# rohitgandikota/sliders

Hardware: AMD Instinct MI355X
Metric: UNet denoise steps/sec (SDXL rank-4 text slider) (higher is better)
Workload: dtype bf16; 1 GPU; sdxl text slider rank=4 alpha=1 noxattn+c3lier, 1024x1024, batch 1 (CFG pair), DDIM-50 partial denoise k~U{1..49} + 4 predictions + backward + AdamW; bench_step=one training iteration, prompt_pairs=8, parallelism=dp1

## Files before the change

### sliders_amd/csrc/lora.hip

```cpp
#include "common.h"
#include "../../include/sliders_hip.h"

namespace {

struct AddrArgs {
    const __bf16* a0; const __bf16* a1;
    int lda0, lda1, ca0, ca1;
    int mode, hs, ws, src_xform, stride, ho, wo;
};

template <int RMAX, int LPR>
__global__ __launch_bounds__(256) void skinny_kernel(AddrArgs A, const __bf16* __restrict__ w,
                                                     const __bf16* __restrict__ bias, void* out,
                                                     int M, int R, int K, int ldo, int out_kind, int kmajor) {
    const int tid = threadIdx.x;
    const int sub = tid & (LPR - 1);
    const int m = blockIdx.x * (256 / LPR) + tid / LPR;
    const bool active = m < M;
    const int mm = active ? m : M - 1;
    float acc[RMAX];
#pragma unroll
    for (int r = 0; r < RMAX; ++r) acc[r] = 0.f;
    const int cin = A.ca0 + A.ca1;

// ... 7 lines not shown
                for (int h = 0; h < 4; ++h) {
                    const bf16x8 wv = *(const bf16x8*)(w + (long)k * 4 + h * 8);
#pragma unroll
                    for (int r = 0; r < 4; ++r) {
                        acc[r] += xf[2 * h] * (float)wv[r];
                        acc[r] += xf[2 * h + 1] * (float)wv[4 + r];
                    }
                }
            }
            return;
        }
        bf16x8 wv[RMAX];
#pragma unroll
        for (int r = 0; r < RMAX; ++r) wv[r] = *(const bf16x8*)(w + (long)(r < R ? r : 0) * K + k);
#pragma unroll
        for (int r = 0; r < RMAX; ++r) {
            if (r < R) {
#pragma unroll
                for (int e = 0; e < 8; ++e) acc[r] += xf[e] * (float)wv[r][e];
            }
        }
    };

    if (A.mode == 0) {
        auto src_of = [&](int k) {
            const int kc = k < K ? k : 0;
            return kc < A.ca0 ? A.a0 + (long)mm * A.lda0 + kc : A.a1 + (long)mm * A.lda1 + (kc - A.ca0);
        };
        bf16x8 cur = *(const bf16x8*)src_of(sub * 8);
        for (int k = sub * 8; k < K; k += LPR * 8) {
            const bf16x8 nxt = *(const bf16x8*)src_of(k + LPR * 8);
            fma_chunk(cur, k);
            cur = nxt;
        }
    } else {
        const int hw = A.ho * A.wo;
        const int b = mm / hw;
        const int rem = mm - b * hw;
        const int oy = rem / A.wo, ox = rem - oy * A.wo;
        const int sh = A.src_xform ? 1 : 0;
        const int HL = A.hs << sh, WL = A.ws << sh;
        for (int tap = 0; tap < 9; ++tap) {
            const int ky = tap / 3, kx = tap - ky * 3;
            const int iy = oy * A.stride + ky - 1, ix = ox * A.stride + kx - 1;
            bool ok = (iy >= 0) & (iy < HL) & (ix >= 0) & (ix < WL);
            if (A.src_xform == 2) ok = ok & (((iy | ix) & 1) == 0);
            if (!ok) continue;
            const long pix = ((long)b * A.hs + (iy >> sh)) * A.ws + (ix >> sh);
            auto src_of = [&](int c) {
                const int cc = c < cin ? c : 0;
                return cc < A.ca0 ? A.a0 + pix * A.lda0 + cc : A.a1 + pix * A.lda1 + (cc - A.ca0);
            };
            bf16x8 cur = *(const bf16x8*)src_of(sub * 8);
            for (int c = sub * 8; c < cin; c += LPR * 8) {
                const bf16x8 nxt = *(const bf16x8*)src_of(c + LPR * 8);
                fma_chunk(cur, tap * cin + c);
                cur = nxt;
            }
        }
    }
#pragma unroll
    for (int r = 0; r < RMAX; ++r) {
#pragma unroll
        for (int o = LPR / 2; o > 0; o >>= 1) acc[r] += __shfl_xor(acc[r], o, 64);
    }
    if (active && sub == 0) {
        if (out_kind == 0) {
            float* o = (float*)out + (long)m * ldo;
#pragma unroll
            for (int r = 0; r < RMAX; ++r)
                if (r < R) o[r] = acc[r] + (bias ? (float)bias[r] : 0.f);
        } else {
            const int hw = A.ho * A.wo;
            const int b = m / hw;
            const int rem = m - b * hw;
            __bf16* o = (__bf16*)out;
#pragma unroll
            for (int r = 0; r < RMAX; ++r)
                if (r < R) o[((long)b * R + r) * hw + rem] = (__bf16)(acc[r] + (bias ? (float)bias[r] : 0.f));
        }
    }
}

__global__ __launch_bounds__(256) void gemv_kernel(const slh_gemv_desc d) {
    const int lane = threadIdx.x & 63;
    const int n = blockIdx.x * 4 + (threadIdx.x >> 6);
    if (n >= d.N) return;
    const __bf16* x = (const __bf16*)d.x;
    const __bf16* w = (const __bf16*)d.w + (long)n * d.K;
    float acc[8];
#pragma unroll
    for (int b = 0; b < 8; ++b) acc[b] = 0.f;
    for (int k = lane * 8; k < d.K; k += 512) {
        const bf16x8 wv = *(const bf16x8*)(w + k);
        bf16x8 xv[8];
#pragma unroll
        for (int b = 0; b < 8; ++b) xv[b] = *(const bf16x8*)(x + (long)(b < d.nb ? b : d.nb - 1) * d.ldx + k);
        float wf[8];
#pragma unroll
        for (int e = 0; e < 8; ++e) wf[e] = (float)wv[e];
#pragma unroll
        for (int b = 0; b < 8; ++b) {
            if (b < d.nb) {
#pragma unroll
                for (int e = 0; e < 8; ++e) {
                    float xe = (float)xv[b][e];
                    if (d.in_act == 1) xe = round_bf16(silu_f(xe));
                    acc[b] += xe * wf[e];
                }
            }
        }
    }
#pragma unroll
    for (int b = 0; b < 8; ++b) acc[b] = wave_sum(acc[b]);
    if (lane == 0) {
        const float bias = d.bias ? (float)((const __bf16*)d.bias)[n] : 0.f;
        float up[4] = {0.f, 0.f, 0.f, 0.f};
        float ls = 0.f;
        int tcol = 0;
        if (d.lora_t) {
            ls = *d.lora_scale;
            tcol = d.lora_tcol ? d.lora_tcol[n] : 0;
            const bf16x4 u = *(const bf16x4*)((const __bf16*)d.lora_up + (long)n * 4);
#pragma unroll
            for (int r = 0; r < 4; ++r) up[r] = (float)u[r];
        }
        for (int b = 0; b < d.nb; ++b) {
            float v = acc[b] + bias;
            if (d.lora_t) {
                const float* t = d.lora_t + (long)b * d.ld_t + tcol;
                v += ls * (t[0] * up[0] + t[1] * up[1] + t[2] * up[2] + t[3] * up[3]);
            }
            if (d.addend) v = round_bf16(v) + (float)((const __bf16*)d.addend)[(long)b * d.ld_add + n];
            if (d.out_f32) ((float*)d.y)[(long)b * d.ldy + n] = v;
            else ((__bf16*)d.y)[(long)b * d.ldy + n] = (__bf16)v;
        }
    }
}

struct WgradArgs {
    AddrArgs A;
    const float* v; float* out; const float* scale;
    int M, R, ldv, ldo, rows_per_block, rmajor, vgroup_cols;
    float* ws; unsigned* ticket;
};

template <int R>
__device__ __forceinline__ void wgrad_body(const WgradArgs& p, const int bx, const int by, const int bz, const long slab_id = 0,
                                           const int slab_step = 0, const long ticket_id = 0, const int splits = 1) {
    __shared__ float red[4][32][8 * R + 1];
    __shared__ int last_flag;
    const int cx = threadIdx.x & 31, ry = threadIdx.x >> 5;
    const int C = p.A.ca0 + p.A.ca1;
    const int c = (bx * 32 + cx) * 8;
    const bool cvalid = c < C;
    const int tap = bz;
    const int m_begin = by * p.rows_per_block;
    const int m_end = min(p.M, m_begin + p.rows_per_block);
    float acc[8][R];
#pragma unroll
    for (int e = 0; e < 8; ++e)
#pragma unroll
        for (int r = 0; r < R; ++r) acc[e][r] = 0.f;
    const int voff = p.vgroup_cols > 0 ? 4 * (c / p.vgroup_cols) : 0;
    const int sh = p.A.src_xform ? 1 : 0;
    const int HL = p.A.hs << sh, WL = p.A.ws << sh;
    const int ky = tap / 3, kx = tap - ky * 3;
    const int hw = p.A.ho * p.A.wo;
    if (cvalid) {
        for (int m = m_begin + ry; m < m_end; m += 8) {
            const __bf16* src;
            if (p.A.mode == 0) {
                src = c < p.A.ca0 ? p.A.a0 + (long)m * p.A.lda0 + c : p.A.a1 + (long)m * p.A.lda1 + (c - p.A.ca0);
            } else {
                const int b = m / hw;
                const int rem = m - b * hw;
                const int oy = rem / p.A.wo, ox = rem - oy * p.A.wo;
                const int iy = oy * p.A.stride + ky - 1, ix = ox * p.A.stride + kx - 1;
                bool ok = (iy >= 0) & (iy < HL) & (ix >= 0) & (ix < WL);
                if (p.A.src_xform == 2) ok = ok & (((iy | ix) & 1) == 0);
                if (!ok) continue;
                const long pix = ((long)b * p.A.hs + (iy >> sh)) * p.A.ws + (ix >> sh);
                src = c < p.A.ca0 ? p.A.a0 + pix * p.A.lda0 + c : p.A.a1 + pix * p.A.lda1 + (c - p.A.ca0);
            }
            const bf16x8 z = *(const bf16x8*)src;
            float vv[R];
#pragma unroll
            for (int r = 0; r < R; ++r) vv[r] = p.v[(long)m * p.ldv + voff + r];
#pragma unroll
            for (int e = 0; e < 8; ++e) {
                const float ze = (float)z[e];
#pragma unroll
                for (int r = 0; r < R; ++r) acc[e][r] += ze * vv[r];
            }
        }
    }
#pragma unroll
    for (int e = 0; e < 8; ++e)
#pragma unroll
        for (int r = 0; r < R; ++r) {
            acc[e][r] += __shfl_xor(acc[e][r], 32, 64);
            if ((threadIdx.x & 32) == 0) red[threadIdx.x >> 6][cx][e * R + r] = acc[e][r];
        }
    __syncthreads();
    const float s = *p.scale;
    if (p.ws != nullptr) {
        constexpr int PER = 32 * 8 * R;
        const __amdgpu_buffer_rsrc_t slabs = __builtin_amdgcn_make_buffer_rsrc(p.ws + slab_id * PER - (long)by * slab_step * PER, 0,
                                                                              (int)((long)splits * slab_step * PER * 4), 0x00020000);
#pragma unroll
        for (int q = 0; q < PER / 1024; ++q) {
            const int idx = (q * 256 + threadIdx.x) * 4;
            f32x4 t4;
#pragma unroll
            for (int u = 0; u < 4; ++u) {
                const int ccx = (idx + u) / (8 * R), er = (idx + u) - ccx * (8 * R);
                float t = 0.f;
#pragma unroll
// ... 45 lines not shown
    }
}

template <int R>
__global__ __launch_bounds__(256) void wgrad_kernel(const WgradArgs p) {
    wgrad_body<R>(p, blockIdx.x, blockIdx.y, blockIdx.z, ((long)blockIdx.z * gridDim.y + blockIdx.y) * gridDim.x + blockIdx.x,
                  (int)gridDim.x, (long)blockIdx.z * gridDim.x + blockIdx.x, (int)gridDim.y);
}

struct WgradGeom { int gx, splits, taps, rows_per_block; };
__host__ __device__ inline WgradGeom wgrad_geom(int C, int M, int mode, int kind) {
    WgradGeom g;
    g.gx = (C / 8 + 31) / 32;
    g.taps = mode == 1 ? 9 : 1;
    const int blocks_xz = g.gx * g.taps;
    const int target = kind == 0 ? 768 : 256;
    int splits = kind == 2 ? (M + 511) / 512 : (target + blocks_xz - 1) / blocks_xz;
    const int max_splits = (M + 63) / 64, min_splits = kind == 2 ? 1 : (M + 1023) / 1024;
    if (splits > max_splits) splits = max_splits;
    if (splits < min_splits) splits = min_splits;
    if (splits < 1) splits = 1;
    g.splits = splits;
    g.rows_per_block = ((M + splits - 1) / splits + 7) / 8 * 8;
    return g;
}

__host__ __device__ inline void wgrad_args(WgradArgs& p, const slh_wgrad_desc& d) {
    p.A.a0 = (const __bf16*)d.z0; p.A.a1 = (const __bf16*)d.z1;
    p.A.lda0 = d.ldz0; p.A.lda1 = d.ldz1; p.A.ca0 = d.c0; p.A.ca1 = d.c1; p.A.mode = d.mode;
    p.A.hs = d.hs; p.A.ws = d.ws; p.A.src_xform = d.src_xform; p.A.stride = d.stride; p.A.ho = d.ho; p.A.wo = d.wo;
    p.v = d.v; p.out = d.out; p.scale = d.scale;
    p.M = d.M; p.R = d.R; p.ldv = d.ldv; p.ldo = d.ldo;
    p.rmajor = d.out_rmajor;
    p.vgroup_cols = d.vgroup_cols;
    p.ws = d.slabs; p.ticket = (unsigned*)d.tickets;
    p.rows_per_block = wgrad_geom(d.c0 + d.c1, d.M, d.mode, d.slabs ? 1 : 0).rows_per_block;
}

__device__ __forceinline__ int batch_find(const int* prefix, int n, int bid) {
    int lo = 0, hi = n;
    while (hi - lo > 1) {
        const int mid = (lo + hi) >> 1;
        if (prefix[mid] <= bid) lo = mid; else hi = mid;
    }
    return lo;
}

template <int R>
__global__ __launch_bounds__(256) void wgrad_batch_kernel(const slh_wgrad_desc* table, const int* prefix, int n, float* ws, unsigned* ticket) {
    const int bid = blockIdx.x;
    const int pi = __builtin_amdgcn_readfirstlane(batch_find(prefix, n, bid));
    const slh_wgrad_desc d = table[pi];
    WgradArgs p;
    wgrad_args(p, d);
    p.ws = ws; p.ticket = ticket;
    const WgradGeom g = wgrad_geom(d.c0 + d.c1, d.M, d.mode, ws ? 2 : 0);
    p.rows_per_block = g.rows_per_block;
    const int local = bid - prefix[pi];
    const int bx = local % g.gx, rest = local / g.gx;
    const int by = rest % g.splits, bz = rest / g.splits;
    wgrad_body<R>(p, bx, by, bz, bid, g.gx, (long)prefix[pi] + (long)bz * g.splits * g.gx + bx, g.splits);
}

}

static int fill_addr(AddrArgs& A, const void* a0, const void* a1, int lda0, int lda1, int ca0, int ca1, int mode,
                     int hs, int ws, int src_xform, int stride, int ho, int wo) {
    A.a0 = (const __bf16*)a0; A.a1 = (const __bf16*)a1;
    A.lda0 = lda0; A.lda1 = lda1; A.ca0 = ca0; A.ca1 = ca1; A.mode = mode;
    A.hs = hs; A.ws = ws; A.src_xform = src_xform; A.stride = stride; A.ho = ho; A.wo = wo;
    return 0;
}

struct skinny_form { int rmax, lpr, grid; };
static skinny_form skinny_choose(int M, int R) {
    skinny_form f;
    f.rmax = R <= 4 ? 4 : R <= 12 ? 12 : 16;
    f.lpr = M <= 16384 ? 64 : 16;
    const int rows = 256 / f.lpr;
    f.grid = (M + rows - 1) / rows;
    return f;
}

extern "C" int slh_skinny(const slh_skinny_desc* d, slh_stream_t stream) {
    SLH_CHECK(d && d->a0 && d->w && d->out, "slh_skinny: null pointer");
    SLH_CHECK(d->M > 0 && d->R > 0 && d->R <= 16 && d->K > 0, "slh_skinny: bad shape");
    SLH_CHECK(d->ca0 % 8 == 0 && d->ca1 % 8 == 0 && d->lda0 % 8 == 0 && d->lda1 % 8 == 0 && d->K % 8 == 0,
              "slh_skinny: 16-byte alignment");
    SLH_CHECK((d->a1 != nullptr) == (d->ca1 > 0), "slh_skinny: a1/ca1 mismatch");
    const int cin = d->ca0 + d->ca1;
    if (d->mode == 0) SLH_CHECK(cin == d->K, "slh_skinny: dense K mismatch");
    else {
        SLH_CHECK(d->mode == 1 && d->K == 9 * cin, "slh_skinny: conv K mismatch");
        SLH_CHECK(d->M == d->batch * d->ho * d->wo, "slh_skinny: conv M mismatch");
        SLH_CHECK(d->stride == 1 || d->stride == 2, "slh_skinny: stride");
    }
    if (d->out_kind == 1) SLH_CHECK(d->mode == 1, "slh_skinny: NCHW output needs conv geometry");
    if (d->w_kmajor) SLH_CHECK(d->R == 4 && d->mode == 0 && !d->bias, "slh_skinny: w_kmajor needs dense R=4");
    AddrArgs A;
    fill_addr(A, d->a0, d->a1, d->lda0, d->lda1, d->ca0, d->ca1, d->mode, d->hs, d->ws, d->src_xform, d->stride,
              d->ho, d->wo);
    hipStream_t s = (hipStream_t)stream;
    const skinny_form f = skinny_choose(d->M, d->R);
#define SLH_SKINNY_LAUNCH(RM, LPR)                                                                                 \
    do {                                                                                                           \
        if (slh_name_mode()) slh_name_record("skinny<%d,%d>", RM, LPR);                                            \
        else                                                                                                       \
            hipLaunchKernelGGL((skinny_kernel<RM, LPR>), dim3(f.grid), dim3(256), 0, s, A, (const __bf16*)d->w,    \
                               (const __bf16*)d->bias, d->out, d->M, d->R, d->K, d->ldo, d->out_kind, d->w_kmajor); \
    } while (0)
#define SLH_SKINNY_ROWS(RM)                                                                                        \
    do {                                                                                                           \
        if (f.lpr == 64) SLH_SKINNY_LAUNCH(RM, 64);                                                                \
        else SLH_SKINNY_LAUNCH(RM, 16);                                                                            \
    } while (0)
    if (f.rmax == 4) SLH_SKINNY_ROWS(4);
    else if (f.rmax == 12) SLH_SKINNY_ROWS(12);
    else SLH_SKINNY_ROWS(16);
#undef SLH_SKINNY_ROWS
#undef SLH_SKINNY_LAUNCH
    SLH_LAUNCH_CHECK("slh_skinny");
    return 0;
}

extern "C" int slh_skinny_kernel_name(const slh_skinny_desc* d, char* buf, int cap) {
    SLH_CHECK(buf && cap >= 32, "slh_skinny_kernel_name: buffer");
    slh_name_sink_set(buf, cap);
    const int rc = slh_skinny(d, nullptr);
    slh_name_sink_set(nullptr, 0);
    if (rc == 0 && !buf[0]) { slh_set_error("slh_skinny_kernel_name: internal: no launch site recorded a name"); return -3; }
    return rc;
}

extern "C" int slh_gemv(const slh_gemv_desc* d, slh_stream_t stream) {
    SLH_CHECK(d && d->x && d->w && d->y, "slh_gemv: null pointer");
    SLH_CHECK(d->nb >= 1 && d->nb <= 8 && d->N > 0 && d->K > 0 && d->K % 8 == 0 && d->ldx % 8 == 0,
              "slh_gemv: bad shape nb=%d N=%d K=%d", d->nb, d->N, d->K);
    if (d->lora_t) SLH_CHECK(d->lora_up && d->lora_scale, "slh_gemv: lora pointers");
    hipLaunchKernelGGL(gemv_kernel, dim3((d->N + 3) / 4), dim3(256), 0, (hipStream_t)stream, *d);
    SLH_LAUNCH_CHECK("slh_gemv");
    return 0;
}

static int wgrad_check(const slh_wgrad_desc* d, bool ptrs = true) {
    SLH_CHECK(d, "slh_lora_wgrad: null descriptor");
    if (ptrs) SLH_CHECK(d->z0 && d->v && d->out && d->scale, "slh_lora_wgrad: null pointer");
    SLH_CHECK(d->R == 4 || d->R == 12, "slh_lora_wgrad: R must be 4 or 12");
    SLH_CHECK(d->c0 % 8 == 0 && d->c1 % 8 == 0 && d->ldz0 % 8 == 0 && d->ldz1 % 8 == 0, "slh_lora_wgrad: alignment");
    if (ptrs) SLH_CHECK((d->z1 != nullptr) == (d->c1 > 0), "slh_lora_wgrad: z1/c1 mismatch");
    SLH_CHECK(d->M > 0 && d->c0 + d->c1 > 0, "slh_lora_wgrad: empty problem");
    if (d->mode == 1) SLH_CHECK(d->M == d->batch * d->ho * d->wo, "slh_lora_wgrad: conv M mismatch");
    if (d->vgroup_cols > 0)
        SLH_CHECK(d->vgroup_cols % 8 == 0 && (d->c0 + d->c1) % d->vgroup_cols == 0 && d->R == 4,
                  "slh_lora_wgrad: vgroup_cols %d needs a multiple of 8 that divides C = %d, and R = 4 (R = %d)", d->vgroup_cols,
                  d->c0 + d->c1, d->R);
    SLH_CHECK(d->vgroup_cols >= 0, "slh_lora_wgrad: negative vgroup_cols");
    return 0;
}

extern "C" int slh_lora_wgrad(const slh_wgrad_desc* d, slh_stream_t stream) {
    if (wgrad_check(d)) return -1;
    WgradArgs p;
    wgrad_args(p, *d);
    SLH_CHECK((d->slabs != nullptr) == (d->tickets != nullptr), "slh_lora_wgrad: slabs and tickets come together");
    const WgradGeom g = wgrad_geom(d->c0 + d->c1, d->M, d->mode, d->slabs ? 1 : 0);
    dim3 grid(g.gx, g.splits, g.taps);
    hipStream_t s = (hipStream_t)stream;
    if (d->R == 4) hipLaunchKernelGGL(wgrad_kernel<4>, grid, dim3(256), 0, s, p);
    else hipLaunchKernelGGL(wgrad_kernel<12>, grid, dim3(256), 0, s, p);
    SLH_LAUNCH_CHECK("slh_lora_wgrad");
    return 0;
}

extern "C" int slh_lora_wgrad_blocks(const slh_wgrad_desc* d) {
    if (wgrad_check(d, false)) return -1;
    const WgradGeom g = wgrad_geom(d->c0 + d->c1, d->M, d->mode, d->slabs ? 2 : 0);
    return g.gx * g.splits * g.taps;
}

extern "C" int slh_lora_wgrad_single_blocks(const slh_wgrad_desc* d) {
    if (wgrad_check(d, false)) return -1;
    const WgradGeom g = wgrad_geom(d->c0 + d->c1, d->M, d->mode, 1);
    return g.gx * g.splits * g.taps;
}

extern "C" int slh_lora_wgrad_geometry(const slh_wgrad_desc* d, int kind, int32_t* out4) {
    if (wgrad_check(d, false)) return -1;
    SLH_CHECK(kind >= 0 && kind <= 2 && out4, "slh_lora_wgrad_geometry: kind must be 0, 1 or 2");
    const WgradGeom g = wgrad_geom(d->c0 + d->c1, d->M, d->mode, kind);
    out4[0] = g.gx; out4[1] = g.splits; out4[2] = g.taps; out4[3] = g.rows_per_block;
    return 0;
}

extern "C" int slh_lora_wgrad_batch(const slh_batch_desc* d, slh_stream_t stream) {
    SLH_CHECK(d && d->table && d->prefix && d->n > 0 && d->total > 0, "slh_lora_wgrad_batch: empty batch / null pointer");
    SLH_CHECK(d->arg == 4 || d->arg == 12, "slh_lora_wgrad_batch: arg must be the common R (4 or 12)");
    SLH_CHECK((d->slabs != nullptr) == (d->tickets != nullptr), "slh_lora_wgrad_batch: slabs and tickets come together");
    hipStream_t s = (hipStream_t)stream;
    if (d->arg == 4)
        hipLaunchKernelGGL(wgrad_batch_kernel<4>, dim3(d->total), dim3(256), 0, s, (const slh_wgrad_desc*)d->table, d->prefix, d->n,
                           (float*)d->slabs, (unsigned*)d->tickets);
    else
        hipLaunchKernelGGL(wgrad_batch_kernel<12>, dim3(d->total), dim3(256), 0, s, (const slh_wgrad_desc*)d->table, d->prefix, d->n,
                           (float*)d->slabs, (unsigned*)d->tickets);
    SLH_LAUNCH_CHECK("slh_lora_wgrad_batch");
    return 0;
}

namespace {
__global__ __launch_bounds__(256) void lora_conv_dgrad_kernel(const slh_lora_cdgrad_desc d) {
    const int nchunk = d.cin / 8;
    const long gid = (long)blockIdx.x * blockDim.x + threadIdx.x;
    const long total = (long)d.batch * d.hl * d.wl * nchunk;
    if (gid >= total) return;
    const int chunk = (int)(gid % nchunk);
    const long pix = gid / nchunk;
    const int hw = d.hl * d.wl;
    const int b = (int)(pix / hw);
    const int rem = (int)(pix - (long)b * hw);
    const int iy = rem / d.wl, ix = rem - iy * d.wl;
    const int c = chunk * 8;
    const __bf16* A = (const __bf16*)d.a_down;
// ... 117 lines not shown
```

### sliders_amd/csrc/ops.hip

```cpp
#include "common.h"
#include "../../include/sliders_hip.h"

namespace {

__global__ void tembed_kernel(const slh_tembed_desc d) {
    const int idx = blockIdx.x * blockDim.x + threadIdx.x;
    const int per = d.n_vals * d.dim;
    if (idx >= d.nb * per) return;
    const int b = idx / per;
    const int rem = idx - b * per;
    const int j = rem / d.dim;
    const int i = rem - j * d.dim;
    const int half = d.dim / 2;
    const int fi = i < half ? i : i - half;
    const float exponent = (-9.210340371976184f * (float)fi) / (float)half;
    const float arg = d.vals[b * d.n_vals + j] * expf(exponent);
    const float v = i < half ? cosf(arg) : sinf(arg);
    ((__bf16*)d.out)[(long)b * d.ldo + d.col0 + rem] = (__bf16)v;
}

constexpr int CONVIN_ITERS = 8;
__global__ void conv_in_kernel(const slh_convin_desc d, int nchunk, int ppb) {
    extern __shared__ __attribute__((aligned(16))) char cin_smem[];
    __bf16* sw = (__bf16*)cin_smem;
    const int K = 9 * d.cin;
    for (int i = threadIdx.x; i < K * d.cout; i += blockDim.x) {
        const int co = i / K, k = i - co * K;
        sw[k * d.cout + co] = ((const __bf16*)d.w)[i];
    }
    __syncthreads();
    const int chunk = threadIdx.x % nchunk, pl = threadIdx.x / nchunk;
    const int hw = d.h * d.wd;
    const long npix = (long)d.batch * hw;
    float bias[8];
#pragma unroll
    for (int e = 0; e < 8; ++e) bias[e] = d.bias ? (float)((const __bf16*)d.bias)[chunk * 8 + e] : 0.f;
    for (int it = 0; it < CONVIN_ITERS; ++it) {
        const long pix = ((long)blockIdx.x * CONVIN_ITERS + it) * ppb + pl;
        if (pix >= npix) break;
        const int b = (int)(pix / hw);
        const int rem = (int)(pix - (long)b * hw);
        const int oy = rem / d.wd, ox = rem - oy * d.wd;
        const __bf16* x = (const __bf16*)d.x + (long)b * d.cin * hw;
        float acc[8];
#pragma unroll
        for (int e = 0; e < 8; ++e) acc[e] = bias[e];
        if (d.cin <= 4) {
            __bf16 xin[9][4];
            bool tin[9];
#pragma unroll
            for (int tap = 0; tap < 9; ++tap) {
                const int iy = oy + tap / 3 - 1, ix = ox + tap % 3 - 1;
                tin[tap] = iy >= 0 && iy < d.h && ix >= 0 && ix < d.wd;
                const int cy = iy < 0 ? 0 : (iy >= d.h ? d.h - 1 : iy), cx = ix < 0 ? 0 : (ix >= d.wd ? d.wd - 1 : ix);
#pragma unroll
                for (int ci = 0; ci < 4; ++ci) xin[tap][ci] = x[(long)(ci < d.cin ? ci : 0) * hw + cy * d.wd + cx];
            }
#pragma unroll
            for (int tap = 0; tap < 9; ++tap) {
                if (!tin[tap]) continue;
#pragma unroll
                for (int ci = 0; ci < 4; ++ci) {
                    if (ci >= d.cin) break;
                    const float xv = (float)xin[tap][ci];
                    const bf16x8 wv = *(const bf16x8*)(sw + (tap * d.cin + ci) * d.cout + chunk * 8);
#pragma unroll
                    for (int e = 0; e < 8; ++e) acc[e] += xv * (float)wv[e];
                }
            }
        } else {
            for (int tap = 0; tap < 9; ++tap) {
                const int iy = oy + tap / 3 - 1, ix = ox + tap % 3 - 1;
                if (iy < 0 || iy >= d.h || ix < 0 || ix >= d.wd) continue;
                for (int ci = 0; ci < d.cin; ++ci) {
                    const float xv = (float)x[(long)ci * hw + iy * d.wd + ix];
                    const bf16x8 wv = *(const bf16x8*)(sw + (tap * d.cin + ci) * d.cout + chunk * 8);
#pragma unroll
                    for (int e = 0; e < 8; ++e) acc[e] += xv * (float)wv[e];
                }
            }
        }
        bf16x8 o;
#pragma unroll
        for (int e = 0; e < 8; ++e) o[e] = (__bf16)acc[e];
        *(bf16x8*)((__bf16*)d.y + pix * d.ldy + chunk * 8) = o;
    }
}

__global__ __launch_bounds__(256) void ew_kernel(const slh_ew_desc d) {
    const int nchunk = d.C / 8;
    const long gid = (long)blockIdx.x * blockDim.x + threadIdx.x;
    if (gid >= (long)d.M * nchunk) return;
    const int chunk = (int)(gid % nchunk);
    const long m = gid / nchunk;
    const int c = chunk * 8;
    const __bf16* A = (const __bf16*)d.a;
    const __bf16* B = (const __bf16*)d.b;
    __bf16* O = (__bf16*)d.out;
    if (d.op == SLH_EW_COPY) {
        *(bf16x8*)(O + m * d.ldo + c) = *(const bf16x8*)(A + m * d.lda + c);
    } else if (d.op == SLH_EW_ADD) {
        const bf16x8 x = *(const bf16x8*)(A + m * d.lda + c);
        const bf16x8 y = *(const bf16x8*)(B + m * d.ldb + c);
        bf16x8 o;
#pragma unroll
        for (int e = 0; e < 8; ++e) o[e] = (__bf16)((float)x[e] + (float)y[e]);
        *(bf16x8*)(O + m * d.ldo + c) = o;
    } else if (d.op == SLH_EW_GEGLU_FWD || d.op == SLH_EW_GEGLU_BWD) {
        const int jb = c >> 5, j = c & 31;
        const __bf16* pa = A + m * d.lda + jb * 64 + j;
        const bf16x8 hv = *(const bf16x8*)pa;
        const bf16x8 gv = *(const bf16x8*)(pa + 32);
        if (d.op == SLH_EW_GEGLU_FWD) {
            bf16x8 o;
#pragma unroll
            for (int e = 0; e < 8; ++e) o[e] = (__bf16)((float)hv[e] * round_bf16(gelu_erf_fast_f((float)gv[e])));
            *(bf16x8*)(O + m * d.ldo + c) = o;
        } else {
            const bf16x8 dy = *(const bf16x8*)(B + m * d.ldb + c);
            bf16x8 dh, dg;
#pragma unroll
            for (int e = 0; e < 8; ++e) {
                const float g = (float)gv[e], hh = (float)hv[e], dd = (float)dy[e];
                const float cdf = 0.5f * (1.f + erff(g * 0.70710678118654752f));
                const float pdf = 0.3989422804014327f * __expf(-0.5f * g * g);
                dh[e] = (__bf16)(dd * round_bf16(g * cdf));
                dg[e] = (__bf16)(round_bf16(dd * hh) * (cdf + g * pdf));
            }
            __bf16* po = O + m * d.ldo + jb * 64 + j;
            *(bf16x8*)po = dh;
            *(bf16x8*)(po + 32) = dg;
        }
    } else if (d.op == SLH_EW_UPSAMPLE_BWD) {
        const int w = d.iarg, hw = d.iarg2;
        const long b = m / hw;
        const int rem = (int)(m - b * hw);
        const int y = rem / w, x = rem - y * w;
        const long base = (b * 4 * hw + (long)(2 * y) * (2 * w) + 2 * x);
        float acc[8];
#pragma unroll
        for (int e = 0; e < 8; ++e) acc[e] = 0.f;
#pragma unroll
        for (int q = 0; q < 4; ++q) {
            const long row = base + (q >> 1) * (2 * w) + (q & 1);
            const bf16x8 v = *(const bf16x8*)(A + row * d.lda + c);
#pragma unroll
            for (int e = 0; e < 8; ++e) acc[e] += (float)v[e];
        }
        bf16x8 o;
#pragma unroll
        for (int e = 0; e < 8; ++e) o[e] = (__bf16)acc[e];
        *(bf16x8*)(O + m * d.ldo + c) = o;
    }
}

__global__ __launch_bounds__(256) void colsum_kernel(const slh_ew_desc d) {
    __shared__ float red[8][33][8];
    const int cx = threadIdx.x & 31, ry = threadIdx.x >> 5;
    const int c = (blockIdx.x * 32 + cx) * 8;
    const int hw = d.iarg2;
    const int b = blockIdx.z;
    const int r0 = blockIdx.y * 512, r1 = min(hw, r0 + 512);
    float acc[8];
#pragma unroll
    for (int e = 0; e < 8; ++e) acc[e] = 0.f;
    if (c < d.C) {
        for (int r = r0 + ry; r < r1; r += 8) {
            const bf16x8 v = *(const bf16x8*)((const __bf16*)d.a + ((long)b * hw + r) * d.lda + c);
// ... 69 lines not shown
        }
    }
    sq = wave_sum(sq);
    __shared__ float part[16];
    if ((threadIdx.x & 63) == 0) part[threadIdx.x >> 6] = sq;
    __syncthreads();
    if (threadIdx.x == 0) {
        float t = 0.f;
#pragma unroll
        for (int w = 0; w < 16; ++w) t += part[w];
        *d.loss += t / (float)d.n;
    }
}

__global__ __launch_bounds__(256) void adamw_kernel(const slh_adamw_desc d, float decay, float bc2_sqrt,
                                                    float step_size, float w1, float beta2, float w2, float eps) {
    const long i = (long)blockIdx.x * blockDim.x + threadIdx.x;
    if (i >= d.n) return;
    __bf16* P = (__bf16*)d.param; __bf16* M1 = (__bf16*)d.exp_avg; __bf16* M2 = (__bf16*)d.exp_avg_sq;
    const float g = round_bf16(d.grad[i] * d.grad_scale);
    float p = round_bf16((float)P[i] * decay);
    float m = (float)M1[i];
    m = round_bf16(m + w1 * (g - m));
    float v = round_bf16((float)M2[i] * beta2);
    v = round_bf16(v + w2 * (g * g));
    float den = round_bf16(sqrtf(v));
    den = round_bf16(den / bc2_sqrt);
    den = round_bf16(den + eps);
    p = round_bf16(p + (-step_size) * (m / den));
    P[i] = (__bf16)p; M1[i] = (__bf16)m; M2[i] = (__bf16)v;
}

__global__ __launch_bounds__(256) void adamw_f32_kernel(const slh_adamw_desc d, float decay, float bc2_sqrt,
                                                        float neg_step_size, float w1, float beta2, float w2, float eps) {
    const long i = (long)blockIdx.x * blockDim.x + threadIdx.x;
    if (i >= d.n) return;
    float* P = (float*)d.param; float* M1 = (float*)d.exp_avg; float* M2 = (float*)d.exp_avg_sq;
    const float g = d.grad_scale == 1.0f ? d.grad[i] : d.grad[i] * d.grad_scale;
    float p = P[i] * decay;
    float m = M1[i];
    m = __builtin_fmaf(w1, g - m, m);
    float v = M2[i] * beta2;
    v = __builtin_fmaf(w2, g * g, v);
    float den = __builtin_sqrtf(v);
    den = den / bc2_sqrt;
    den = den + eps;
    p = __builtin_fmaf(neg_step_size, m / den, p);
    P[i] = p; M1[i] = m; M2[i] = v;
    ((__bf16*)d.param_lo)[i] = (__bf16)p;
}

__global__ __launch_bounds__(256) void lion_kernel(const slh_lion_desc d, float decay, float b1, float w1, float b2,
                                                   float w2, float neg_lr) {
    const long i = (long)blockIdx.x * blockDim.x + threadIdx.x;
    if (i >= d.n) return;
    __bf16* P = (__bf16*)d.param; __bf16* M = (__bf16*)d.exp_avg;
    const float g = round_bf16(d.grad[i] * d.grad_scale);
    float p = round_bf16((float)P[i] * decay);
    const float m0 = (float)M[i];
    float u = round_bf16(m0 * b1);
    u = round_bf16(u + w1 * g);
    const float sg = u > 0.f ? 1.f : (u < 0.f ? -1.f : 0.f);
    p = round_bf16(p + neg_lr * sg);
    float m = round_bf16(m0 * b2);
    m = round_bf16(m + w2 * g);
    P[i] = (__bf16)p; M[i] = (__bf16)m;
}

}

extern "C" int slh_timestep_embed(const slh_tembed_desc* d, slh_stream_t stream) {
    SLH_CHECK(d && d->vals && d->out && d->dim % 2 == 0 && d->nb > 0 && d->n_vals > 0, "slh_timestep_embed: bad desc");
    const int total = d->nb * d->n_vals * d->dim;
    hipLaunchKernelGGL(tembed_kernel, dim3((total + 255) / 256), dim3(256), 0, (hipStream_t)stream, *d);
    SLH_LAUNCH_CHECK("slh_timestep_embed");
    return 0;
}

extern "C" int slh_conv_in(const slh_convin_desc* d, slh_stream_t stream) {
    SLH_CHECK(d && d->x && d->w && d->y, "slh_conv_in: null pointer");
    SLH_CHECK(d->cout % 8 == 0 && d->ldy % 8 == 0 && d->cin > 0 && d->cin <= 16, "slh_conv_in: bad shape");
    const int nchunk = d->cout / 8;
    SLH_CHECK(nchunk <= 256 && 9 * d->cin * d->cout * 2 <= 64 * 1024, "slh_conv_in: weights must fit 64 KB of LDS");
    const int ppb = 256 / nchunk;
    const long npix = (long)d->batch * d->h * d->wd;
    const long per_block = (long)ppb * CONVIN_ITERS;
    hipLaunchKernelGGL(conv_in_kernel, dim3((unsigned)((npix + per_block - 1) / per_block)), dim3(nchunk * ppb),
                       9 * d->cin * d->cout * 2, (hipStream_t)stream, *d, nchunk, ppb);
    SLH_LAUNCH_CHECK("slh_conv_in");
    return 0;
}

extern "C" int slh_elementwise(const slh_ew_desc* d, slh_stream_t stream) {
    SLH_CHECK(d && d->a && d->out, "slh_elementwise: null pointer");
    SLH_CHECK(d->C % 8 == 0 && d->lda % 8 == 0 && d->ldo % 4 == 0, "slh_elementwise: alignment");
    hipStream_t s = (hipStream_t)stream;
    if (d->op == SLH_EW_COLSUM) {
        SLH_CHECK(d->iarg2 > 0 && d->M % d->iarg2 == 0, "slh_elementwise: colsum rows per sample");
        dim3 grid((d->C / 8 + 31) / 32, (d->iarg2 + 511) / 512, d->M / d->iarg2);
        hipLaunchKernelGGL(colsum_kernel, grid, dim3(256), 0, s, *d);
    } else {
        if (d->op == SLH_EW_ADD || d->op == SLH_EW_GEGLU_BWD) SLH_CHECK(d->b && d->ldb % 8 == 0, "slh_elementwise: operand b");
        if (d->op == SLH_EW_GEGLU_FWD || d->op == SLH_EW_GEGLU_BWD) SLH_CHECK(d->C % 32 == 0, "slh_elementwise: geglu C");
        if (d->op == SLH_EW_UPSAMPLE_BWD) SLH_CHECK(d->iarg > 0 && d->iarg2 > 0, "slh_elementwise: upsample dims");
        const long total = (long)d->M * (d->C / 8);
        hipLaunchKernelGGL(ew_kernel, dim3((unsigned)((total + 255) / 256)), dim3(256), 0, s, *d);
    }
    SLH_LAUNCH_CHECK("slh_elementwise");
    return 0;
}

namespace {
__global__ __launch_bounds__(256) void gather16_kernel(const unsigned short* src, const int* idx, unsigned short* out, long n) {
    const long i = (long)blockIdx.x * blockDim.x + threadIdx.x;
    if (i >= n) return;
    const int j = idx[i];
    out[i] = j < 0 ? (unsigned short)0 : src[j];
}
}

extern "C" int slh_gather16(const slh_gather16_desc* d, slh_stream_t stream) {
    SLH_CHECK(d && d->src && d->idx && d->out && d->n > 0, "slh_gather16: null pointer / empty");
    hipLaunchKernelGGL(gather16_kernel, dim3((unsigned)((d->n + 255) / 256)), dim3(256), 0, (hipStream_t)stream,
                       (const unsigned short*)d->src, d->idx, (unsigned short*)d->out, (long)d->n);
    SLH_LAUNCH_CHECK("slh_gather16");
    return 0;
}

extern "C" int slh_cfg_ddim(const slh_cfg_ddim_desc* d, slh_stream_t stream) {
    SLH_CHECK(d && d->eps && d->out && (d->x || !d->do_step), "slh_cfg_ddim: null pointer");
    const long n = (long)d->nb * d->chw;
    hipLaunchKernelGGL(cfg_ddim_kernel, dim3((unsigned)((n + 255) / 256)), dim3(256), 0, (hipStream_t)stream, *d);
    SLH_LAUNCH_CHECK("slh_cfg_ddim");
    return 0;
}

extern "C" int slh_guidance_loss(const slh_loss_desc* d, slh_stream_t stream) {
    SLH_CHECK(d && d->target && d->positive && d->neutral && d->uncond && d->loss, "slh_guidance_loss: null pointer");
    hipLaunchKernelGGL(loss_kernel, dim3(1), dim3(1024), 0, (hipStream_t)stream, *d);
    SLH_LAUNCH_CHECK("slh_guidance_loss");
    return 0;
}

extern "C" int slh_adamw(const slh_adamw_desc* d, slh_stream_t stream) {
    SLH_CHECK(d && d->param && d->exp_avg && d->exp_avg_sq && d->grad && d->step >= 1, "slh_adamw: bad desc");
    const double bc1 = 1.0 - pow(d->beta1, (double)d->step);
    const double bc2 = 1.0 - pow(d->beta2, (double)d->step);
    const float step_size = (float)(d->lr / bc1);
    const float bc2_sqrt = (float)sqrt(bc2);
    const float decay = (float)(1.0 - d->lr * d->weight_decay);
    if (d->f32_state) {
        SLH_CHECK(d->param_lo && ((uintptr_t)d->param & 3) == 0, "slh_adamw: f32_state needs param_lo (the bf16 copy the kernels read)");
        hipLaunchKernelGGL(adamw_f32_kernel, dim3((unsigned)((d->n + 255) / 256)), dim3(256), 0, (hipStream_t)stream, *d,
                           decay, bc2_sqrt, -step_size, (float)(1.0 - d->beta1), (float)d->beta2, (float)(1.0 - d->beta2), (float)d->eps);
        SLH_LAUNCH_CHECK("slh_adamw (fp32 state)");
        return 0;
    }
    hipLaunchKernelGGL(adamw_kernel, dim3((unsigned)((d->n + 255) / 256)), dim3(256), 0, (hipStream_t)stream, *d,
                       decay, bc2_sqrt, step_size, (float)(1.0 - d->beta1), (float)d->beta2, (float)(1.0 - d->beta2),
                       (float)d->eps);
    SLH_LAUNCH_CHECK("slh_adamw");
    return 0;
}

extern "C" int slh_lion(const slh_lion_desc* d, slh_stream_t stream) {
    SLH_CHECK(d && d->param && d->exp_avg && d->grad && d->n > 0, "slh_lion: bad desc");
// ... 7 lines not shown
```

Baseline: 44.98 steps/s.

## Add MFMA kernels for LoRA skinny conv and conv_in, retune GEMV

Adds an MFMA-based kernel for the rank-4 LoRA down-projection over 3x3 conv inputs. It stages padded weights in LDS and prefetches the next channel chunk into registers. It also adds an MFMA path for the 4-channel conv_in layer, with weights and bias held in registers. The GEMV kernel is templated on batch count and rows per wave, with K unrolled by three. Together these aim to replace scalar FMA loops with matrix-core instructions and cut redundant loads, at the cost of more registers, extra edge-case handling and new code paths to keep correct.

```diff
diff --git a/sliders_amd/csrc/lora.hip b/sliders_amd/csrc/lora.hip
--- a/sliders_amd/csrc/lora.hip
+++ b/sliders_amd/csrc/lora.hip
@@ -113,58 +113,179 @@
     }
 }
 
+constexpr int SKMF_U = 10;
+constexpr int SKMF_PX = 14;
+__global__ __launch_bounds__(256) void skinny_conv_mfma_kernel(AddrArgs A, const __bf16* __restrict__ w,
+                                                               const __bf16* __restrict__ bias, void* out,
+                                                               int R, int K, int ldo, int out_kind, int ldw, int spr, int nwaves) {
+    extern __shared__ __attribute__((aligned(16))) char skmf_smem[];
+    __bf16* sw = (__bf16*)skmf_smem;
+    float* sp = (float*)(skmf_smem + 4 * ldw * 2) + (threadIdx.x >> 6) * 256;
+    const int kch = K >> 3, total = 4 * kch;
+    for (int i0 = threadIdx.x; i0 < total; i0 += 256 * 8) {
+        bf16x8 v[8];
+#pragma unroll
+        for (int u = 0; u < 8; ++u) {
+            const int i = i0 + 256 * u < total ? i0 + 256 * u : i0;
+            const int r = i / kch, c = i - r * kch;
+            v[u] = *(const bf16x8*)(w + (long)(r < R ? r : 0) * K + c * 8);
+        }
+#pragma unroll
+        for (int u = 0; u < 8; ++u) {
+            const int i = i0 + 256 * u;
+            if (i < total) {
+                const int r = i / kch, c = i - r * kch;
+                bf16x8 z;
+#pragma unroll
+                for (int e = 0; e < 8; ++e) z[e] = r < R ? v[u][e] : (__bf16)0.f;
+                *(bf16x8*)(sw + r * ldw + c * 8) = z;
+            }
+        }
+    }
+    __syncthreads();
+    const int lane = threadIdx.x & 63;
+    const int gwv = blockIdx.x * 4 + (threadIdx.x >> 6);
+    const bool live = gwv < nwaves;
+    const int wv = live ? gwv : nwaves - 1;
+    const int p = lane & 15, q = lane >> 4;
+    const int cin = A.ca0 + A.ca1;
+    const int row = wv / spr, ox0 = (wv - row * spr) * SKMF_PX;
+    const int b = row / A.hs, oy = row - b * A.hs;
+    const int ix = ox0 - 1 + p;
+    const int cx = ix < 0 ? 0 : (ix >= A.ws ? A.ws - 1 : ix);
+    const bool xok = live & (ix >= 0) & (ix < A.ws);
+    const int nck = (cin + 32 * SKMF_U - 1) / (32 * SKMF_U);
+    const int T = 3 * nck;
+    const int kxl = (p >> 2) < 3 ? (p >> 2) : 0;
+    const __bf16* swl = sw + (p & 3) * ldw + kxl * cin + 8 * q;
+
+    auto request = [&](int it, bf16x8 (&dst)[SKMF_U], bool& ok) {
+        const int ky = it / nck, c0 = (it - ky * nck) * (32 * SKMF_U);
+        const int iy = oy + ky - 1;
+        ok = xok & (iy >= 0) & (iy < A.hs);
+        const int cy = iy < 0 ? 0 : (iy >= A.hs ? A.hs - 1 : iy);
+        const long pix = ((long)b * A.hs + cy) * A.ws + cx;
+#pragma unroll
+        for (int u = 0; u < SKMF_U; ++u) {
+            const int cu = c0 + 32 * u;
+            const int c = (cu < cin ? cu : 0) + 8 * q;
+            dst[u] = *(const bf16x8*)(c < A.ca0 ? A.a0 + pix * A.lda0 + c : A.a1 + pix * A.lda1 + (c - A.ca0));
+        }
+    };
+
+    f32x4 acc[2] = {f32x4{0.f, 0.f, 0.f, 0.f}, f32x4{0.f, 0.f, 0.f, 0.f}};
+    bf16x8 cur[SKMF_U], nxt[SKMF_U];
+    bool cur_ok, nxt_ok;
+    request(0, cur, cur_ok);
+    for (int it = 0; it < T; ++it) {
+        request(it + 1 < T ? it + 1 : it, nxt, nxt_ok);
+        const int ky = it / nck, c0 = (it - ky * nck) * (32 * SKMF_U);
+#pragma unroll
+        for (int u = 0; u < SKMF_U; ++u) {
+            const int cu = c0 + 32 * u;
+            if (cu < cin) {
+                bf16x8 a;
+#pragma unroll
+                for (int e = 0; e < 8; ++e) a[e] = cur_ok ? cur[u][e] : (__bf16)0.f;
+                const bf16x8 wv8 = *(const bf16x8*)(swl + ky * 3 * cin + cu);
+                acc[u & 1] = __builtin_amdgcn_mfma_f32_16x16x32_bf16(a, wv8, acc[u & 1], 0, 0, 0);
+            }
+        }
+#pragma unroll
+        for (int u = 0; u < SKMF_U; ++u) cur[u] = nxt[u];
+        cur_ok = nxt_ok;
+    }
+#pragma unroll
+    for (int i = 0; i < 4; ++i) sp[(4 * q + i) * 16 + p] = acc[0][i] + acc[1][i];
+    __syncthreads();
+    const int o = 1 + (lane >> 2), r = lane & 3;
+    const int ox = ox0 + o - 1;
+    if (live && lane < 4 * SKMF_PX && r < R && ox < A.ws) {
+        const float v = sp[(o - 1) * 16 + r] + sp[o * 16 + 4 + r] + sp[(o + 1) * 16 + 8 + r] + (bias ? (float)bias[r] : 0.f);
+        const int hw = A.hs * A.ws;
+        const int rem = oy * A.ws + ox;
+        if (out_kind == 0) ((float*)out)[((long)b * hw + rem) * ldo + r] = v;
+        else ((__bf16*)out)[((long)b * R + r) * hw + rem] = (__bf16)v;
+    }
+}
+
+constexpr int GEMV_KU = 3;
+template <int NB, int RN>
 __global__ __launch_bounds__(256) void gemv_kernel(const slh_gemv_desc d) {
     const int lane = threadIdx.x & 63;
-    const int n = blockIdx.x * 4 + (threadIdx.x >> 6);
-    if (n >= d.N) return;
+    const int n0 = (blockIdx.x * 4 + (threadIdx.x >> 6)) * RN;
+    if (n0 >= d.N) return;
     const __bf16* x = (const __bf16*)d.x;
-    const __bf16* w = (const __bf16*)d.w + (long)n * d.K;
-    float acc[8];
-#pragma unroll
-    for (int b = 0; b < 8; ++b) acc[b] = 0.f;
-    for (int k = lane * 8; k < d.K; k += 512) {
-        const bf16x8 wv = *(const bf16x8*)(w + k);
-        bf16x8 xv[8];
-#pragma unroll
-        for (int b = 0; b < 8; ++b) xv[b] = *(const bf16x8*)(x + (long)(b < d.nb ? b : d.nb - 1) * d.ldx + k);
-        float wf[8];
-#pragma unroll
-        for (int e = 0; e < 8; ++e) wf[e] = (float)wv[e];
-#pragma unroll
-        for (int b = 0; b < 8; ++b) {
-            if (b < d.nb) {
-#pragma unroll
-                for (int e = 0; e < 8; ++e) {
-                    float xe = (float)xv[b][e];
-                    if (d.in_act == 1) xe = round_bf16(silu_f(xe));
-                    acc[b] += xe * wf[e];
+    const __bf16* w = (const __bf16*)d.w;
+    float acc[RN][NB];
+#pragma unroll
+    for (int r = 0; r < RN; ++r)
+#pragma unroll
+        for (int b = 0; b < NB; ++b) acc[r][b] = 0.f;
+    for (int k0 = lane * 8; k0 < d.K; k0 += 512 * GEMV_KU) {
+        bf16x8 wv[RN][GEMV_KU], xv[NB][GEMV_KU];
+#pragma unroll
+        for (int u = 0; u < GEMV_KU; ++u) {
+            const int k = k0 + 512 * u;
+            const int kc = k < d.K ? k : k0;
+#pragma unroll
+            for (int r = 0; r < RN; ++r) wv[r][u] = *(const bf16x8*)(w + (long)(n0 + r < d.N ? n0 + r : n0) * d.K + kc);
+#pragma unroll
+            for (int b = 0; b < NB; ++b) xv[b][u] = *(const bf16x8*)(x + (long)(b < d.nb ? b : d.nb - 1) * d.ldx + kc);
+        }
+#pragma unroll
+        for (int u = 0; u < GEMV_KU; ++u) {
+            if (k0 + 512 * u < d.K) {
+#pragma unroll
+                for (int b = 0; b < NB; ++b) {
+                    if (b < d.nb) {
+                        float xf[8];
+#pragma unroll
+                        for (int e = 0; e < 8; ++e) {
+                            xf[e] = (float)xv[b][u][e];
+                            if (d.in_act == 1) xf[e] = round_bf16(silu_f(xf[e]));
+                        }
+#pragma unroll
+                        for (int r = 0; r < RN; ++r)
+#pragma unroll
+                            for (int e = 0; e < 8; ++e) acc[r][b] += xf[e] * (float)wv[r][u][e];
+                    }
                 }
             }
         }
     }
 #pragma unroll
-    for (int b = 0; b < 8; ++b) acc[b] = wave_sum(acc[b]);
-    if (lane == 0) {
-        const float bias = d.bias ? (float)((const __bf16*)d.bias)[n] : 0.f;
-        float up[4] = {0.f, 0.f, 0.f, 0.f};
-        float ls = 0.f;
-        int tcol = 0;
-        if (d.lora_t) {
-            ls = *d.lora_scale;
-            tcol = d.lora_tcol ? d.lora_tcol[n] : 0;
-            const bf16x4 u = *(const bf16x4*)((const __bf16*)d.lora_up + (long)n * 4);
-#pragma unroll
-            for (int r = 0; r < 4; ++r) up[r] = (float)u[r];
-        }
-        for (int b = 0; b < d.nb; ++b) {
-            float v = acc[b] + bias;
+    for (int r = 0; r < RN; ++r)
+#pragma unroll
+        for (int b = 0; b < NB; ++b) acc[r][b] = wave_sum(acc[r][b]);
+#pragma unroll
+    for (int r = 0; r < RN; ++r) {
+        const int n = n0 + r;
+        if (lane == r && n < d.N) {
+            const float bias = d.bias ? (float)((const __bf16*)d.bias)[n] : 0.f;
+            float up[4] = {0.f, 0.f, 0.f, 0.f};
+            float ls = 0.f;
+            int tcol = 0;
             if (d.lora_t) {
-                const float* t = d.lora_t + (long)b * d.ld_t + tcol;
-                v += ls * (t[0] * up[0] + t[1] * up[1] + t[2] * up[2] + t[3] * up[3]);
-            }
-            if (d.addend) v = round_bf16(v) + (float)((const __bf16*)d.addend)[(long)b * d.ld_add + n];
-            if (d.out_f32) ((float*)d.y)[(long)b * d.ldy + n] = v;
-            else ((__bf16*)d.y)[(long)b * d.ldy + n] = (__bf16)v;
+                ls = *d.lora_scale;
+                tcol = d.lora_tcol ? d.lora_tcol[n] : 0;
+                const bf16x4 u = *(const bf16x4*)((const __bf16*)d.lora_up + (long)n * 4);
+#pragma unroll
+                for (int j = 0; j < 4; ++j) up[j] = (float)u[j];
+            }
+#pragma unroll
+            for (int b = 0; b < NB; ++b) {
+                if (b < d.nb) {
+                    float v = acc[r][b] + bias;
+                    if (d.lora_t) {
+                        const float* t = d.lora_t + (long)b * d.ld_t + tcol;
+                        v += ls * (t[0] * up[0] + t[1] * up[1] + t[2] * up[2] + t[3] * up[3]);
+                    }
+                    if (d.addend) v = round_bf16(v) + (float)((const __bf16*)d.addend)[(long)b * d.ld_add + n];
+                    if (d.out_f32) ((float*)d.y)[(long)b * d.ldy + n] = v;
+                    else ((__bf16*)d.y)[(long)b * d.ldy + n] = (__bf16)v;
+                }
+            }
         }
     }
 }
@@ -376,6 +497,21 @@
     return f;
 }
 
+#ifndef SLH_SKINNY_MFMA_MIN_M
+#define SLH_SKINNY_MFMA_MIN_M 4096
+#endif
+static int skinny_mfma_ldw(int K) {
+    int ldw = K;
+    while ((ldw / 2) % 64 != 16) ldw += 8;
+    return ldw;
+}
+static bool skinny_takes_mfma(const slh_skinny_desc* d) {
+    const int cin = d->ca0 + d->ca1;
+    return d->mode == 1 && d->R <= 4 && !d->w_kmajor && d->stride == 1 && d->src_xform == 0 && d->ho == d->hs && d->wo == d->ws &&
+           d->ca0 % 32 == 0 && d->ca1 % 32 == 0 && cin >= 32 && 4 * skinny_mfma_ldw(d->K) * 2 <= 60 * 1024 &&
+           d->M >= SLH_SKINNY_MFMA_MIN_M;
+}
+
 extern "C" int slh_skinny(const slh_skinny_desc* d, slh_stream_t stream) {
     SLH_CHECK(d && d->a0 && d->w && d->out, "slh_skinny: null pointer");
     SLH_CHECK(d->M > 0 && d->R > 0 && d->R <= 16 && d->K > 0, "slh_skinny: bad shape");
@@ -395,6 +531,17 @@
     fill_addr(A, d->a0, d->a1, d->lda0, d->lda1, d->ca0, d->ca1, d->mode, d->hs, d->ws, d->src_xform, d->stride,
               d->ho, d->wo);
     hipStream_t s = (hipStream_t)stream;
+    if (skinny_takes_mfma(d)) {
+        const int ldw = skinny_mfma_ldw(d->K);
+        const int spr = (d->ws + SKMF_PX - 1) / SKMF_PX;
+        const int nwaves = d->batch * d->hs * spr;
+        if (slh_name_mode()) slh_name_record("skinny_conv_mfma<%d>", SKMF_U);
+        else
+            hipLaunchKernelGGL(skinny_conv_mfma_kernel, dim3((nwaves + 3) / 4), dim3(256), 4 * ldw * 2 + 4 * 1024, s, A,
+                               (const __bf16*)d->w, (const __bf16*)d->bias, d->out, d->R, d->K, d->ldo, d->out_kind, ldw, spr, nwaves);
+        SLH_LAUNCH_CHECK("slh_skinny");
+        return 0;
+    }
     const skinny_form f = skinny_choose(d->M, d->R);
 #define SLH_SKINNY_LAUNCH(RM, LPR)                                                                                 \
     do {                                                                                                           \
@@ -431,7 +578,17 @@
     SLH_CHECK(d->nb >= 1 && d->nb <= 8 && d->N > 0 && d->K > 0 && d->K % 8 == 0 && d->ldx % 8 == 0,
               "slh_gemv: bad shape nb=%d N=%d K=%d", d->nb, d->N, d->K);
     if (d->lora_t) SLH_CHECK(d->lora_up && d->lora_scale, "slh_gemv: lora pointers");
-    hipLaunchKernelGGL(gemv_kernel, dim3((d->N + 3) / 4), dim3(256), 0, (hipStream_t)stream, *d);
+    const int rn = d->N >= 8192 ? 4 : 1;
+    const int grid = (d->N + 4 * rn - 1) / (4 * rn);
+#define SLH_GEMV_LAUNCH(NB)                                                                                      \
+    do {                                                                                                         \
+        if (rn == 4) hipLaunchKernelGGL((gemv_kernel<NB, 4>), dim3(grid), dim3(256), 0, (hipStream_t)stream, *d); \
+        else hipLaunchKernelGGL((gemv_kernel<NB, 1>), dim3(grid), dim3(256), 0, (hipStream_t)stream, *d);        \
+    } while (0)
+    if (d->nb <= 2) SLH_GEMV_LAUNCH(2);
+    else if (d->nb <= 4) SLH_GEMV_LAUNCH(4);
+    else SLH_GEMV_LAUNCH(8);
+#undef SLH_GEMV_LAUNCH
     SLH_LAUNCH_CHECK("slh_gemv");
     return 0;
 }
diff --git a/sliders_amd/csrc/ops.hip b/sliders_amd/csrc/ops.hip
--- a/sliders_amd/csrc/ops.hip
+++ b/sliders_amd/csrc/ops.hip
@@ -84,6 +84,94 @@
 #pragma unroll
         for (int e = 0; e < 8; ++e) o[e] = (__bf16)acc[e];
         *(bf16x8*)((__bf16*)d.y + pix * d.ldy + chunk * 8) = o;
+    }
+}
+
+constexpr int CONVIN_MF_TILES = 5;
+constexpr int CONVIN_MF_WAVES = 2048;
+__global__ __launch_bounds__(256) void conv_in_mfma_kernel(const slh_convin_desc d, int groups, int spr, int nstrips, int wpg) {
+    const int lane = threadIdx.x & 63;
+    const int gw = blockIdx.x * 4 + (threadIdx.x >> 6);
+    if (gw >= groups * wpg) return;
+    const int group = gw % groups;
+    const int n = lane & 31, h = lane >> 5;
+    const __bf16* w = (const __bf16*)d.w;
+    const __bf16* bias = (const __bf16*)d.bias;
+    const int cl = 16 * ((n >> 2) & 1) + 4 * (n >> 3) + (n & 3);
+    bf16x8 wf[CONVIN_MF_TILES][3], bb[CONVIN_MF_TILES][2];
+#pragma unroll
+    for (int t = 0; t < CONVIN_MF_TILES; ++t) {
+        const int c0 = (group * CONVIN_MF_TILES + t) * 32;
+        const int co = c0 + cl;
+        const bool cok = co < d.cout;
+        const __bf16* wr = w + (long)(cok ? co : 0) * 36;
+        bf16x4 q[3][2];
+#pragma unroll
+        for (int s = 0; s < 3; ++s)
+#pragma unroll
+            for (int u = 0; u < 2; ++u) {
+                const int tap = 4 * s + 2 * h + u;
+                q[s][u] = *(const bf16x4*)(wr + (tap < 9 ? tap : 8) * 4);
+            }
+#pragma unroll
+        for (int s = 0; s < 3; ++s)
+#pragma unroll
+            for (int j = 0; j < 8; ++j)
+                wf[t][s][j] = (cok && 4 * s + 2 * h + (j >> 2) < 9) ? q[s][j >> 2][j & 3] : (__bf16)0.f;
+#pragma unroll
+        for (int u = 0; u < 2; ++u) {
+            const int cb = c0 + 16 * h + 8 * u;
+            const bool bok = cb < d.cout;
+#pragma unroll
+            for (int j = 0; j < 8; ++j) bb[t][u][j] = (__bf16)0.f;
+            if (bias) {
+                const bf16x8 v = *(const bf16x8*)(bias + (bok ? cb : 0));
+#pragma unroll
+                for (int j = 0; j < 8; ++j) bb[t][u][j] = bok ? v[j] : (__bf16)0.f;
+            }
+        }
+    }
+    const int hw = d.h * d.wd;
+    for (int st = gw / groups; st < nstrips; st += wpg) {
+        const int row = st / spr, ox = (st - row * spr) * 32 + n;
+        const int b = row / d.h, oy = row - b * d.h;
+        const __bf16* x = (const __bf16*)d.x + (long)b * 4 * hw;
+        __bf16 xin[3][2][4];
+        bool tin[3][2];
+#pragma unroll
+        for (int s = 0; s < 3; ++s)
+#pragma unroll
+            for (int u = 0; u < 2; ++u) {
+                const int tap = 4 * s + 2 * h + u;
+                const int tc = tap < 9 ? tap : 8;
+                const int iy = oy + tc / 3 - 1, ix = ox + tc % 3 - 1;
+                tin[s][u] = tap < 9 && iy >= 0 && iy < d.h && ix >= 0 && ix < d.wd;
+                const int cy = iy < 0 ? 0 : (iy >= d.h ? d.h - 1 : iy), cx = ix < 0 ? 0 : (ix >= d.wd ? d.wd - 1 : ix);
+#pragma unroll
+                for (int ci = 0; ci < 4; ++ci) xin[s][u][ci] = x[(long)ci * hw + cy * d.wd + cx];
+            }
+        bf16x8 xf[3];
+#pragma unroll
+        for (int s = 0; s < 3; ++s)
+#pragma unroll
+            for (int j = 0; j < 8; ++j) xf[s][j] = tin[s][j >> 2] ? xin[s][j >> 2][j & 3] : (__bf16)0.f;
+        __bf16* yrow = (__bf16*)d.y + ((long)row * d.wd + ox) * d.ldy;
+#pragma unroll
+        for (int t = 0; t < CONVIN_MF_TILES; ++t) {
+            f32x16 acc;
+#pragma unroll
+            for (int r = 0; r < 16; ++r) acc[r] = (float)bb[t][r >> 3][r & 7];
+#pragma unroll
+            for (int s = 0; s < 3; ++s) acc = __builtin_amdgcn_mfma_f32_32x32x16_bf16(wf[t][s], xf[s], acc, 0, 0, 0);
+#pragma unroll
+            for (int u = 0; u < 2; ++u) {
+                const int cb = (group * CONVIN_MF_TILES + t) * 32 + 16 * h + 8 * u;
+                bf16x8 o;
+#pragma unroll
+                for (int e = 0; e < 8; ++e) o[e] = (__bf16)acc[8 * u + e];
+                if (ox < d.wd && cb < d.cout) *(bf16x8*)(yrow + cb) = o;
+            }
+        }
     }
 }
 
@@ -319,6 +407,19 @@
     SLH_CHECK(d->cout % 8 == 0 && d->ldy % 8 == 0 && d->cin > 0 && d->cin <= 16, "slh_conv_in: bad shape");
     const int nchunk = d->cout / 8;
     SLH_CHECK(nchunk <= 256 && 9 * d->cin * d->cout * 2 <= 64 * 1024, "slh_conv_in: weights must fit 64 KB of LDS");
+    SLH_CHECK(d->batch > 0 && d->h > 0 && d->wd > 0 && (long)d->batch * d->h * d->wd < (1L << 31), "slh_conv_in: bad image size");
+    const bool mfma = d->cin == 4 && ((uintptr_t)d->w & 7) == 0 && ((uintptr_t)d->y & 15) == 0 && ((uintptr_t)d->bias & 15) == 0;
+    if (mfma) {
+        const int spr = (d->wd + 31) / 32;
+        const int nstrips = d->batch * d->h * spr;
+        const int groups = (d->cout + 32 * CONVIN_MF_TILES - 1) / (32 * CONVIN_MF_TILES);
+        const int cap = CONVIN_MF_WAVES / groups > 0 ? CONVIN_MF_WAVES / groups : 1;
+        const int wpg = nstrips < cap ? nstrips : cap;
+        hipLaunchKernelGGL(conv_in_mfma_kernel, dim3((unsigned)((groups * wpg + 3) / 4)), dim3(256), 0, (hipStream_t)stream, *d,
+                           groups, spr, nstrips, wpg);
+        SLH_LAUNCH_CHECK("slh_conv_in");
+        return 0;
+    }
     const int ppb = 256 / nchunk;
     const long npix = (long)d->batch * d->h * d->wd;
     const long per_block = (long)ppb * CONVIN_ITERS;
```

New measurement: 45.21 steps/s, median of 6. No clear change (+0.5%).
